# autowarefoundation/autoware_vision_pilot

Hardware: NVIDIA H100
Metric: camera frames/sec @1080p multi-task (higher is better)
Workload: dtype f16

## Files before the change

### autoware_vision_pilot_b200/_lib.py

```python
from __future__ import annotations

import ctypes as C
import os

import numpy as np

_HERE = os.path.dirname(os.path.abspath(__file__))
LIB_PATH = os.path.join(_HERE, "lib", "libvp_b200.so")

VPB_F16, VPB_BF16 = 0, 1
ACT_NONE, ACT_GELU, ACT_SILU, ACT_SIGMOID = 0, 1, 2, 3
EPI_STORE, EPI_ADD, EPI_MULADD, EPI_FINAL = 0, 1, 2, 3
FINAL_NONE, FINAL_ARGMAX, FINAL_THRESH, FINAL_EGOLANES = 0, 1, 2, 3
ALGO_TILE, ALGO_LINEAR = 0, 1


class ConvArgs(C.Structure):

    _fields_ = [
        ("dtype", C.c_int),
        ("H", C.c_int), ("W", C.c_int), ("Cin", C.c_int), ("ldi", C.c_int),
        ("Cout", C.c_int), ("taps", C.c_int), ("phases", C.c_int),
        ("act", C.c_int), ("mode", C.c_int), ("final_kind", C.c_int),
        ("inp", C.c_void_p), ("w", C.c_void_p), ("bias", C.c_void_p),
# ... 263 lines not shown
                ("bev_left_coeffs", C.c_double * 6), ("bev_right_coeffs", C.c_double * 6),
                ("bev_center_coeffs", C.c_double * 6),
                ("lane_offset", C.c_double), ("yaw_offset", C.c_double), ("curvature", C.c_double),
                ("bev_lane_offset", C.c_double), ("bev_yaw_offset", C.c_double), ("bev_curvature", C.c_double),
                ("last_valid_width_pixels", C.c_double),
                ("left_valid", C.c_int), ("right_valid", C.c_int), ("path_valid", C.c_int), ("bev_valid", C.c_int),
                ("filt_left_valid", C.c_int), ("filt_right_valid", C.c_int),
                ("left_start", C.c_int * 2), ("right_start", C.c_int * 2),
                ("n_left_pts", C.c_int), ("n_right_pts", C.c_int),
                ("pf_left_coeff", C.c_double * 3), ("pf_right_coeff", C.c_double * 3),
                ("pf_left_cte", C.c_double), ("pf_left_yaw_error", C.c_double),
                ("pf_right_cte", C.c_double), ("pf_right_yaw_error", C.c_double),
                ("pf_cte", C.c_double), ("pf_yaw_error", C.c_double), ("pf_curvature", C.c_double),
                ("pf_lane_width", C.c_double), ("pf_cte_variance", C.c_double), ("pf_yaw_variance", C.c_double),
                ("pf_curv_variance", C.c_double), ("pf_lane_width_variance", C.c_double),
                ("pf_fused_valid", C.c_int), ("pf_ran", C.c_int),
                ("pf_meas", (C.c_double * 2) * 14)]


_lib = None


def lib() -> C.CDLL:
    global _lib
    if _lib is None:
        if not os.path.exists(LIB_PATH):
            raise RuntimeError(
                f"{LIB_PATH} is missing — run `python -c 'import __graft_entry__ as g; g.build()'` "
                "(there is no CPU or PyTorch fallback for the B200 path)")
        _lib = C.CDLL(LIB_PATH)
        _lib.vpb_last_error.restype = C.c_char_p
        _lib.vpb_conv_gemm.argtypes = [C.POINTER(ConvArgs), C.c_void_p]
        _lib.vpb_conv_gemm.restype = C.c_int
    return _lib


def last_error() -> str:
    return lib().vpb_last_error().decode("utf-8", "replace")


def check(rc: int, what: str) -> None:
    if rc != 0:
        raise RuntimeError(f"{what} failed (rc={rc}): {last_error()}")
```

### autoware_vision_pilot_b200/csrc/conv_gemm.cu

```cuda
#include "common.cuh"
#include "conv_gemm.cuh"
#include "ops_internal.h"
#include <cstdio>
#include <cstring>
#include <algorithm>

namespace vpb {

static constexpr int kMma = 256;
static constexpr int kEpilogue = 128;
static constexpr int kThreads = kMma + kEpilogue + 32;
static constexpr int kMaxStages = 8;
static constexpr int kATileBytes = 128 * 128;
static constexpr int kMaxDynSmem = 227 * 1024 - 4096;
__host__ __device__ constexpr int acc_pitch(int bn) { return bn + 4; }
__host__ __device__ constexpr size_t acc_bytes(int bn) { return static_cast<size_t>(128) * acc_pitch(bn) * 4; }

__device__ __forceinline__ void acc_ld16(uint32_t t, uint32_t (&r)[16]) {
  const uint32_t a = t << 2;
#pragma unroll
  for (int i = 0; i < 4; ++i)
    asm volatile("ld.shared.v4.b32 {%0, %1, %2, %3}, [%4];"
                 : "=r"(r[4 * i]), "=r"(r[4 * i + 1]), "=r"(r[4 * i + 2]), "=r"(r[4 * i + 3])
                 : "r"(a + 16u * i)
// ... 179 lines not shown
    uint32_t ra[16];
    acc_ld16(ta, ra);
    finish(ra, sb4, op, rp);
  }
}

template <class E>
__device__ __forceinline__ void epilogue_tile(const ConvKParams& p, uint32_t t_row, int n0,
                                              const float* sbias, const EpiPix& px) {
  const bool whole = !p.split && n0 + p.BN <= p.nlim && p.act2 == ACT_NONE;
  if (whole && p.mode == VPB_EPI_STORE && p.act == ACT_GELU) epilogue_store_fast<E, ACT_GELU>(p, t_row, n0, sbias, px);
  else if (whole && p.mode == VPB_EPI_STORE && p.act == ACT_NONE) epilogue_store_fast<E, ACT_NONE>(p, t_row, n0, sbias, px);
  else if (whole && p.mode == VPB_EPI_STORE && p.act == ACT_SILU) epilogue_store_fast<E, ACT_SILU>(p, t_row, n0, sbias, px);
  else if (whole && p.mode == VPB_EPI_ADD && p.act == ACT_NONE && n0 + p.BN <= p.ldr) epilogue_store_fast<E, ACT_NONE, true>(p, t_row, n0, sbias, px);
  else epilogue_chunks<E>(p, t_row, n0, sbias, px);
}

struct TileCoord { int img, ph, n0, h0, w0; };

__device__ __forceinline__ TileCoord decode_tile(const ConvKParams& p, int tile) {
  TileCoord c;
  c.img = static_cast<int>(fast_div(tile, p.mg_ti));
  const int ti = tile - c.img * p.tiles_img;
  c.ph = static_cast<int>(fast_div(ti, p.mg_tpp));
  const int r = ti - c.ph * (p.tiles_n * p.tiles_h * p.tiles_w);
  const int rn = static_cast<int>(fast_div(r, p.mg_tn));
  const int thi = static_cast<int>(fast_div(rn, p.mg_tw));
  c.n0 = (r - rn * p.tiles_n) * p.BN;
  c.h0 = thi * p.TH;
  c.w0 = (rn - thi * p.tiles_w) * p.TW;
  return c;
}

template <class E, int BN>
__global__ void __launch_bounds__(kThreads, 1)
conv_wgmma_kernel(const __grid_constant__ ConvMaps maps, const ConvKParams p) {
  extern __shared__ uint8_t smem_raw[];
  __shared__ __align__(8) uint64_t bar_full[kMaxStages];
  __shared__ __align__(8) uint64_t bar_empty[kMaxStages];
  __shared__ __align__(8) uint64_t acc_full;
  __shared__ __align__(8) uint64_t acc_empty;
  __shared__ __align__(16) float s_bias[BN];

  constexpr uint32_t kBTileBytes = static_cast<uint32_t>(BN) * 128u;
  constexpr uint32_t kStageBytes = kATileBytes + kBTileBytes;
  constexpr int kPitch = acc_pitch(BN);
  const int warp = threadIdx.x >> 5;
  const int lane = threadIdx.x & 31;
  const uint32_t smem_base = (smem_u32(smem_raw) + 1023u) & ~1023u;
  const uint32_t acc_base = smem_base + static_cast<uint32_t>(p.stages) * kStageBytes;

  if (threadIdx.x == kMma + kEpilogue) {
    tma_prefetch_desc(&maps.A);
    tma_prefetch_desc(&maps.B);
    if (p.kchunks2) { tma_prefetch_desc(&maps.A2); tma_prefetch_desc(&maps.B2); }
    if (p.split) { tma_prefetch_desc(&maps.Alo); tma_prefetch_desc(&maps.Blo); }
    for (int s = 0; s < p.stages; ++s) {
      mbar_init(smem_u32(&bar_full[s]), 1);
      mbar_init(smem_u32(&bar_empty[s]), kMma / 32);
    }
    mbar_init(smem_u32(&acc_full), kMma);
    mbar_init(smem_u32(&acc_empty), kEpilogue);
    fence_mbar_init();
  }
  __syncthreads();
  pdl_launch_dependents();
  pdl_wait();

  const int nseg = p.split ? 3 : 1;
  const int kiters_all = p.upc ? 4 * p.kchunks + 9 * p.kchunks2 : (p.taps * p.kchunks + p.kchunks2) * nseg;

  if (warp == (kMma + kEpilogue) / 32) {
    int stage = 0;
    uint32_t phase = 0;
    auto load_stage = [&](const CUtensorMap* mA, int a0, int a1, int a2, int a3,
                          const CUtensorMap* mB, int b0, int b1, int b2) {
      mbar_wait_quiet(smem_u32(&bar_empty[stage]), phase ^ 1u);
      if (elect_one()) {
        const uint32_t full = smem_u32(&bar_full[stage]);
        const uint32_t sa = smem_base + stage * kStageBytes;
        mbar_arrive_expect_tx(full, kStageBytes);
        tma_load_4d(sa, mA, full, a0, a1, a2, a3);
        tma_load_3d(sa + kATileBytes, mB, full, b0, b1, b2);
      }
      __syncwarp();
      if (++stage == p.stages) { stage = 0; phase ^= 1u; }
    };
    for (int tile = blockIdx.x; tile < p.total_tiles; tile += gridDim.x) {
      const auto [img, ph, n0, h0, w0] = decode_tile(p, tile);
      if (p.upc) {
        const int pa = ph >> 1, pb = ph & 1;
        for (int t = 0; t < 4; ++t) {
          const int oy = (t >> 1) - 1 + pa, ox = (t & 1) - 1 + pb;
          for (int c = 0; c < p.kchunks; ++c)
            load_stage(&maps.A, c * 64, w0 + ox, h0 + oy, img, &maps.B, c * 64, n0, ph * 4 + t);
        }
        for (int t2 = 0; t2 < (p.kchunks2 ? 9 : 0); ++t2) {
          const int dy = t2 / 3, dx = t2 - dy * 3;
          const int u = pa + dy - 1, v = pb + dx - 1;
          for (int c2 = 0; c2 < p.kchunks2; ++c2)
            load_stage(&maps.A2, c2 * 64, 2 * w0 + v, 2 * h0 + u, img, &maps.B2, c2 * 64, n0, t2);
        }
        continue;
      }
      for (int t = 0; t < p.taps; ++t) {
        const int dy = (p.taps == 9) ? (t / 3 - 1) : 0;
        const int dx = (p.taps == 9) ? (t % 3 - 1) : 0;
        const int wsel = p.w_img ? img : (p.phases > 1) ? ph : t;
        for (int c = 0; c < p.kchunks; ++c)
          for (int seg = 0; seg < nseg; ++seg)
            load_stage(seg == 1 ? &maps.Alo : &maps.A, c * 64, w0 * p.stride + dx, h0 * p.stride + dy, img,
                       seg == 2 ? &maps.Blo : &maps.B, c * 64, n0, wsel);
      }
      const int s2 = p.phases > 1 ? 2 : 1;
      for (int c2 = 0; c2 < p.kchunks2; ++c2)
        for (int seg = 0; seg < nseg; ++seg)
          load_stage(seg == 1 ? &maps.A2lo : &maps.A2, c2 * 64, s2 * w0 + (ph & 1), s2 * h0 + (ph >> 1), img,
                     seg == 2 ? &maps.B2lo : &maps.B2, c2 * 64, n0, 0);
    }
  } else if (warp < kMma / 32) {
    const int wg = warp >> 2;
    float* acc_s = reinterpret_cast<float*>(smem_raw + (acc_base - smem_u32(smem_raw)));
    float acc[BN / 2];
    int stage = 0, prev = 0;
    uint32_t phase = 0, acc_phase = 0;
    for (int tile = blockIdx.x; tile < p.total_tiles; tile += gridDim.x) {
      for (int k = 0; k < kiters_all; ++k) {
        mbar_wait_quiet(smem_u32(&bar_full[stage]), phase);
        const uint32_t sa = smem_base + stage * kStageBytes;
        const uint64_t adesc = wgmma_desc_k128(sa + wg * (64 * 128));
        const uint64_t bdesc = wgmma_desc_k128(sa + kATileBytes);
        wgmma_fence();
#pragma unroll
        for (int kk = 0; kk < 4; ++kk)
          Wgmma<E, BN>::mma(acc, adesc + 2 * kk, bdesc + 2 * kk, (k | kk) != 0 ? 1u : 0u);
        wgmma_commit();
        wgmma_wait<1>();
        if (k > 0 && lane == 0) mbar_arrive(smem_u32(&bar_empty[prev]));
        prev = stage;
        if (++stage == p.stages) { stage = 0; phase ^= 1u; }
      }
      wgmma_wait<0>();
      if (lane == 0) mbar_arrive(smem_u32(&bar_empty[prev]));

      mbar_wait_quiet(smem_u32(&acc_empty), acc_phase ^ 1u);
      {
        const int r0 = wg * 64 + (warp & 3) * 16 + (lane >> 2);
        float* a0 = acc_s + r0 * kPitch + 2 * (lane & 3);
#pragma unroll
        for (int j = 0; j < BN / 8; ++j) {
          *reinterpret_cast<float2*>(a0 + 8 * j) = make_float2(acc[4 * j], acc[4 * j + 1]);
          *reinterpret_cast<float2*>(a0 + 8 * kPitch + 8 * j) = make_float2(acc[4 * j + 2], acc[4 * j + 3]);
        }
      }
      mbar_arrive(smem_u32(&acc_full));
      acc_phase ^= 1u;
    }
  } else {
    const int row = threadIdx.x - kMma;
    const int lh = row >> p.tw_shift;
    const int lw = row & (p.TW - 1);
    const int Wo = (p.phases > 1) ? 2 * p.W : p.W;
    const uint32_t t_row = (acc_base >> 2) + static_cast<uint32_t>(row * kPitch);
    uint32_t acc_phase = 0;
    for (int tile = blockIdx.x; tile < p.total_tiles; tile += gridDim.x) {
      const auto [img, ph, n0, h0, w0] = decode_tile(p, tile);
      const int h = h0 + lh, w = w0 + lw;

      named_bar_sync(1, kEpilogue);
      if (row < BN) {
        const int nn = n0 + row;
        s_bias[row] = (p.bias && nn < p.Cout) ? __ldg(p.bias + (p.upc ? 4 * p.Cout : 0) + nn) : 0.f;
      }
      named_bar_sync(1, kEpilogue);
      mbar_wait_quiet(smem_u32(&acc_full), acc_phase);

      const int oh = (p.phases > 1) ? 2 * h + (ph >> 1) : h;
      const int ow = (p.phases > 1) ? 2 * w + (ph & 1) : w;
      EpiPix px;
      px.ok = (h < p.H) && (w < p.W);
      px.ooff = img * p.out_img + static_cast<uint32_t>((oh + p.out_pad) * (Wo + 2 * p.out_pad) + (ow + p.out_pad)) * p.ldo;
      px.roff = img * p.res_img + static_cast<uint32_t>((oh + p.res_pad) * (Wo + 2 * p.res_pad) + (ow + p.res_pad)) * p.ldr;
      px.fpix = static_cast<uint32_t>(h * p.W + w);
      px.img = static_cast<uint32_t>(img);
      if (p.upc) {
        const int pa = ph >> 1, pb = ph & 1;
        const int cy = (pa == 0 && h == 0) ? 0 : (pa == 1 && h == p.H - 1) ? 2 : 1;
        const int cx = (pb == 0 && w == 0) ? 0 : (pb == 1 && w == p.W - 1) ? 2 : 1;
        const int cls = cy * 3 + cx;
        const float* gb = cls != 4 ? p.bias + cls * p.Cout + n0 : nullptr;
        if (p.act == ACT_GELU) epilogue_store_fast<E, ACT_GELU, false, true>(p, t_row, n0, s_bias, px, gb);
        else epilogue_store_fast<E, ACT_NONE, false, true>(p, t_row, n0, s_bias, px, gb);
      } else {
        epilogue_tile<E>(p, t_row, n0, s_bias, px);
      }
      mbar_arrive(smem_u32(&acc_empty));
      acc_phase ^= 1u;
    }
  }
}

__global__ void zero_border_kernel(uint4* out, int H, int W, int ldo, int nlim) {
  pdl_wait();
  out += (static_cast<size_t>(blockIdx.y) * (H + 2) * (W + 2) * ldo) >> 3;
  const int per = nlim >> 3, nb = 2 * (W + 2) + 2 * H;
  for (int i = blockIdx.x * blockDim.x + threadIdx.x; i < nb * per; i += gridDim.x * blockDim.x) {
    const int pix = i / per, v = i - pix * per;
    int y, x;
// ... 72 lines not shown
        q == cudaDriverEntryPointSuccess)
      fn = reinterpret_cast<EncodeTiledFn>(p);
  }
  return fn;
}

static int encode_map(CUtensorMap* m, const char* name, CUtensorMapDataType dt, int rank, const void* base,
                      const cuuint64_t* dims, const cuuint64_t* strides, const cuuint32_t* box, const cuuint32_t* es,
                      CUtensorMapL2promotion l2) {
  const CUresult r = get_encode_fn()(m, dt, rank, const_cast<void*>(base), dims, strides, box, es,
                                     CU_TENSOR_MAP_INTERLEAVE_NONE, CU_TENSOR_MAP_SWIZZLE_128B, l2,
                                     CU_TENSOR_MAP_FLOAT_OOB_FILL_NONE);
  if (r == CUDA_SUCCESS) return VPB_OK;
  vpb_set_error("conv: cuTensorMapEncodeTiled(%s) failed: %d", name, static_cast<int>(r));
  return VPB_ERR_CUDA;
}

int device_sm_count() {
  int dev = 0, n = 0;
  cudaGetDevice(&dev);
  cudaDeviceGetAttribute(&n, cudaDevAttrMultiProcessorCount, dev);
  return n > 0 ? n : 132;
}

static int pick_bn(int Cout, int want) {
  if (want > 0) return want <= 16 ? 16 : want <= 32 ? 32 : want <= 64 ? 64 : 128;
  for (int bn : {128, 64, 32}) {
    if (Cout <= bn && (Cout > bn / 2 || bn == 32)) return bn;
    if (Cout > bn && (Cout + bn - 1) / bn * bn - Cout <= Cout / 4) return bn;
  }
  return 16;
}

int conv_plan_build(const vpb_conv_args* a, ConvPlan* plan) {
  if (!a || !plan) return VPB_ERR_ARG;
  if (a->Cin <= 0 || (a->Cin & 7) || (a->ldi & 7) || a->ldi < a->Cin) {
    vpb_set_error("conv: Cin=%d ldi=%d must be multiples of 8 (ldi >= Cin)", a->Cin, a->ldi);
    return VPB_ERR_ARG;
  }
  const int cstride = a->stride == 2 ? 2 : 1;
  if (a->stride != 0 && a->stride != 1 && a->stride != 2) { vpb_set_error("conv: stride %d unsupported", a->stride); return VPB_ERR_ARG; }
  if (cstride == 2 && (a->algo == VPB_ALGO_LINEAR || a->phases != 1 || a->in_pad || a->in2 || a->in_lo)) {
    vpb_set_error("conv: stride 2 needs the TILE algorithm on an unpadded input, phases = 1, no second input");
    return VPB_ERR_ARG;
  }
  if (a->ldw != 0 && (a->ldw < a->Cin || (a->ldw & 7) || a->algo == VPB_ALGO_LINEAR)) {
    vpb_set_error("conv: ldw=%d must be a multiple of 8 >= Cin (TILE algorithm)", a->ldw);
    return VPB_ERR_ARG;
  }
  if (a->act2 != ACT_NONE && a->act2 != ACT_SILU) { vpb_set_error("conv: act2 supports SiLU only"); return VPB_ERR_ARG; }
  const bool upc = a->taps == 4 && a->phases == 4;
  if (upc && (a->algo == VPB_ALGO_LINEAR || a->in_lo || a->mode != VPB_EPI_STORE || (a->act != ACT_NONE && a->act != ACT_GELU) ||
              !a->bias || (a->Cout & 15) || a->out_slice || cstride != 1 || a->ldw || (a->in2 && a->taps2 != 9))) {
    vpb_set_error("conv: upconv (taps=4, phases=4) needs the TILE algorithm, 16-bit mode, STORE, act NONE|GELU, bias[9][Cout], Cout%%16==0, taps2=9 with in2");
    return VPB_ERR_ARG;
  }
  if (!((a->taps == 9 && a->phases == 1) || (a->taps == 1 && (a->phases == 1 || a->phases == 4)) || upc)) {
    vpb_set_error("conv: unsupported taps=%d phases=%d", a->taps, a->phases);
    return VPB_ERR_ARG;
  }
  const bool lin = a->algo == VPB_ALGO_LINEAR;
  if (lin && (a->taps != 9 || !a->in_pad)) {
    vpb_set_error("conv: the linear-padded algorithm needs a 3x3 conv on a zero-bordered input");
    return VPB_ERR_ARG;
  }
  if (a->mode == VPB_EPI_FINAL) {
    if (a->Cout > 32 || (a->out_cls && a->Cout > 16) || !a->out_f32) {
// ... 71 lines not shown
  }
  p.tiles_n = (a->Cout + p.BN - 1) / p.BN;
  p.kchunks = (a->Cin + 63) / 64;
  p.Cin2 = a->in2 ? a->Cin2 : 0;
  p.kchunks2 = (p.Cin2 + 63) / 64;
  int best_tw = 128; long best_cost = -1;
  for (int tw = 128; tw >= 8; tw >>= 1) {
    const int th = 128 / tw;
    const long cost = static_cast<long>((a->H + th - 1) / th) * ((a->W + tw - 1) / tw);
    if (best_cost < 0 || cost < best_cost) { best_cost = cost; best_tw = tw; }
  }
  p.TW = best_tw; p.TH = 128 / best_tw;
  p.tw_shift = 0; while ((1 << p.tw_shift) < p.TW) ++p.tw_shift;
  p.tiles_h = (a->H + p.TH - 1) / p.TH;
  p.tiles_w = (a->W + p.TW - 1) / p.TW;
  p.tiles_img = p.tiles_h * p.tiles_w * p.tiles_n * p.phases;
  p.total_tiles = p.tiles_img * batch;
  p.mg_ti = fast_div_magic(p.tiles_img);
  {
    const long ho = a->phases == 4 ? 2L * a->H : a->H, wo = a->phases == 4 ? 2L * a->W : a->W;
    p.out_img = static_cast<uint32_t>((ho + 2 * p.out_pad) * (wo + 2 * p.out_pad) * a->ldo);
    p.res_img = static_cast<uint32_t>((ho + 2 * p.res_pad) * (wo + 2 * p.res_pad) * a->ldr);
  }
  const size_t stage_bytes = kATileBytes + static_cast<size_t>(p.BN) * 128;
  p.stages = static_cast<int>(std::min<size_t>(kMaxStages, (kMaxDynSmem - 1024 - acc_bytes(p.BN)) / stage_bytes));
  if (p.stages < 2) { vpb_set_error("conv: no room for the operand ring (BN %d)", p.BN); return VPB_ERR_ARG; }
  plan->smem_bytes = p.stages * stage_bytes + acc_bytes(p.BN) + 1024;
  p.mg_tn = fast_div_magic(p.tiles_n); p.mg_tw = fast_div_magic(p.tiles_w);
  p.mg_tpp = fast_div_magic(p.tiles_n * p.tiles_h * p.tiles_w);
  p.act = a->act; p.mode = a->mode; p.final_kind = a->final_kind;
  p.bias = a->bias; p.out = a->out; p.ldo = a->ldo; p.res = a->res; p.ldr = a->ldr;
  p.out_f32 = a->out_f32; p.out_cls = a->out_cls;
  plan->dtype = a->dtype;
  plan->grid = std::min(p.total_tiles, device_sm_count());
  plan->flops = 2.0 * batch * a->H * a->W * static_cast<double>(a->Cout) * a->phases * (a->Cin * a->taps + p.Cin2 * (upc ? 9 : 1));

  const CUtensorMapDataType dt =
      a->dtype == VPB_BF16 ? CU_TENSOR_MAP_DATA_TYPE_BFLOAT16 : CU_TENSOR_MAP_DATA_TYPE_FLOAT16;
  ConvMaps& m = plan->maps;
  int rc;
  {
    const int pad = p.in_pad;
    const int Hin = (cstride == 2 && a->in_h > 0) ? a->in_h : a->H, Win = (cstride == 2 && a->in_w > 0) ? a->in_w : a->W;
    const size_t pitch = static_cast<size_t>(Win + 2 * pad) * a->ldi * 2;
    const size_t skip = pad * pitch + static_cast<size_t>(pad) * a->ldi * 2;
    const cuuint64_t dims[4] = {static_cast<cuuint64_t>(a->Cin), static_cast<cuuint64_t>(Win),
                                static_cast<cuuint64_t>(Hin), static_cast<cuuint64_t>(batch)};
    const cuuint64_t strides[3] = {static_cast<cuuint64_t>(a->ldi) * 2, pitch, pitch * (Hin + 2 * pad)};
    const cuuint32_t box[4] = {64, static_cast<cuuint32_t>(p.TW * cstride), static_cast<cuuint32_t>(p.TH * cstride), 1};
    const cuuint32_t es[4] = {1, static_cast<cuuint32_t>(cstride), static_cast<cuuint32_t>(cstride), 1};
    if ((rc = encode_map(&m.A, "A", dt, 4, static_cast<const uint8_t*>(a->in) + skip, dims, strides, box, es,
                         CU_TENSOR_MAP_L2_PROMOTION_L2_128B)))
      return rc;
    if (split && (rc = encode_map(&m.Alo, "Alo", dt, 4, static_cast<const uint8_t*>(a->in_lo) + skip, dims, strides, box,
                                  es, CU_TENSOR_MAP_L2_PROMOTION_L2_128B)))
      return rc;
  }
  {
    const size_t ldw = a->ldw > 0 ? a->ldw : a->Cin;
    const cuuint64_t dims[3] = {static_cast<cuuint64_t>(a->Cin), static_cast<cuuint64_t>(a->Cout),
                                static_cast<cuuint64_t>(a->w_img ? batch : a->taps * a->phases)};
    const cuuint64_t strides[2] = {static_cast<cuuint64_t>(ldw) * 2,
                                   a->w_img ? static_cast<cuuint64_t>(a->w_img) * 2 : static_cast<cuuint64_t>(ldw) * 2 * a->Cout};
    const cuuint32_t box[3] = {64, static_cast<cuuint32_t>(p.BN), 1};
    const cuuint32_t es[3] = {1, 1, 1};
    if ((rc = encode_map(&m.B, "B", dt, 3, a->w, dims, strides, box, es, CU_TENSOR_MAP_L2_PROMOTION_L2_256B))) return rc;
    if (split && (rc = encode_map(&m.Blo, "Blo", dt, 3, a->w_lo, dims, strides, box, es, CU_TENSOR_MAP_L2_PROMOTION_L2_256B)))
      return rc;
  }
  if (!split) { m.Alo = m.A; m.Blo = m.B; }
  m.A2 = m.A; m.B2 = m.B; m.A2lo = m.Alo; m.B2lo = m.Blo;
  if (a->in2) {
    const int s2 = a->phases == 4 ? 2 : 1;
    const int pad = a->in2_pad ? 1 : 0;
    const size_t px = static_cast<size_t>(a->ld2) * 2;
    const size_t pitch = static_cast<size_t>(a->W * s2 + 2 * pad) * px;
    const size_t skip = pad * pitch + pad * px;
    const cuuint64_t dims[4] = {static_cast<cuuint64_t>(a->Cin2), static_cast<cuuint64_t>(a->W * s2),
                                static_cast<cuuint64_t>(a->H * s2), static_cast<cuuint64_t>(batch)};
    const cuuint64_t strides[3] = {px, pitch, pitch * (a->H * s2 + 2 * pad)};
    const cuuint32_t box[4] = {64, static_cast<cuuint32_t>(p.TW * s2), static_cast<cuuint32_t>(p.TH * s2), 1};
    const cuuint32_t es[4] = {1, static_cast<cuuint32_t>(s2), static_cast<cuuint32_t>(s2), 1};
    if ((rc = encode_map(&m.A2, "A2", dt, 4, static_cast<const uint8_t*>(a->in2) + skip, dims, strides, box, es,
                         CU_TENSOR_MAP_L2_PROMOTION_L2_128B)))
      return rc;
    if (split && (rc = encode_map(&m.A2lo, "A2lo", dt, 4, static_cast<const uint8_t*>(a->in2_lo) + skip, dims, strides,
                                  box, es, CU_TENSOR_MAP_L2_PROMOTION_L2_128B)))
      return rc;
    const cuuint64_t bd[3] = {static_cast<cuuint64_t>(a->Cin2), static_cast<cuuint64_t>(a->Cout), static_cast<cuuint64_t>(p.upc ? 9 : 1)};
    const cuuint64_t bs[2] = {static_cast<cuuint64_t>(a->Cin2) * 2, static_cast<cuuint64_t>(a->Cin2) * 2 * a->Cout};
    const cuuint32_t bb[3] = {64, static_cast<cuuint32_t>(p.BN), 1};
    const cuuint32_t be[3] = {1, 1, 1};
    if ((rc = encode_map(&m.B2, "B2", dt, 3, a->w2, bd, bs, bb, be, CU_TENSOR_MAP_L2_PROMOTION_L2_256B))) return rc;
    if (split && (rc = encode_map(&m.B2lo, "B2lo", dt, 3, a->w2_lo, bd, bs, bb, be, CU_TENSOR_MAP_L2_PROMOTION_L2_256B)))
      return rc;
  }
  return VPB_OK;
}

static void (*const kConvKernels[2][4])(ConvMaps, ConvKParams) = {
    {conv_wgmma_kernel<F16, 16>, conv_wgmma_kernel<F16, 32>, conv_wgmma_kernel<F16, 64>, conv_wgmma_kernel<F16, 128>},
    {conv_wgmma_kernel<BF16, 16>, conv_wgmma_kernel<BF16, 32>, conv_wgmma_kernel<BF16, 64>, conv_wgmma_kernel<BF16, 128>},
};

int conv_plan_launch(const ConvPlan* plan, cudaStream_t stream) {
  {
    std::lock_guard<std::mutex> g(init_mutex());
    bool* done = device_flag(kInitConv);
    if (!*done) {
      for (const auto& by_bn : kConvKernels)
        for (const auto k : by_bn) VPB_CUDA_OK(cudaFuncSetAttribute(k, cudaFuncAttributeMaxDynamicSharedMemorySize, kMaxDynSmem));
      *done = true;
    }
  }
  const ConvKParams& p = plan->p;
  const auto kernel = kConvKernels[plan->dtype == VPB_BF16][__builtin_ctz(p.BN >> 4)];
  VPB_CUDA_OK(launch_k(kernel, dim3(plan->grid), dim3(kThreads), plan->smem_bytes, stream, plan->maps, p));
  if (p.lin) {
    const int n = (2 * (p.W + 2) + 2 * p.H) * (p.nlim >> 3);
    VPB_CUDA_OK(launch_k(zero_border_kernel, dim3(std::min((n + 255) / 256, 256), p.total_tiles / p.tiles_img), dim3(256), 0, stream,
                         static_cast<uint4*>(p.out), p.H, p.W, p.ldo, p.nlim));
  }
  return VPB_OK;
}

}


extern "C" int vpb_conv_gemm(const vpb_conv_args* a, void* stream) {
  vpb::ConvPlan plan;
  int rc = vpb::conv_plan_build(a, &plan);
  if (rc != VPB_OK) return rc;
  return vpb::conv_plan_launch(&plan, static_cast<cudaStream_t>(stream));
}

extern "C" int vpb_final_tapsum(const float* P, const float* bias, int Cout, int H, int W, int final_kind, float* out,
                                uint8_t* cls, int batch, void* stream) {
  return vpb::final_tapsum_x(P, bias, Cout, H, W, final_kind, out, cls, static_cast<cudaStream_t>(stream), batch);
}
```

### autoware_vision_pilot_b200/csrc/conv_gemm.cuh

```cuda
#pragma once
#include <cuda.h>
#include <cuda_runtime.h>
#include <stdint.h>
#include "../../include/vp_b200_ops.h"

namespace vpb {

struct ConvKParams {
  int H, W, Cin, Cout;
  int taps, phases;
  int TH, TW, tw_shift;
  int BN;
  int tiles_h, tiles_w, tiles_n;
  int total_tiles;
  int tiles_img;
  uint32_t mg_ti;
  uint32_t out_img, res_img;
  int kchunks;
  int Cin2, kchunks2;
  int stages;
  int lin;
  int upc;
  int nlim;
  int stride;
  int act2;
  int split;
  void* out_lo;
  const void* res_lo;
  int in_pad, out_pad, res_pad;
  uint32_t mg_tn, mg_tw, mg_tpp;
  int act, mode, final_kind;
  const float* bias;
  void* out;
  int ldo;
  const void* res;
  int ldr;
  float* out_f32;
  uint8_t* out_cls;
  int w_img;
};

struct ConvMaps {
  CUtensorMap A, B;
  CUtensorMap A2, B2;
  CUtensorMap Alo, Blo, A2lo, B2lo;
};

struct ConvPlan {
  ConvMaps maps;
  ConvKParams p;
  int dtype;
  int grid;
  size_t smem_bytes;
  double flops;
};

int conv_plan_build(const vpb_conv_args* a, ConvPlan* plan);
int conv_plan_launch(const ConvPlan* plan, cudaStream_t stream);
int device_sm_count();

}
```

### autoware_vision_pilot_b200/csrc/engine_common.cu

```cuda
#include "common.cuh"
#include "conv_gemm.cuh"
#include "engine_internal.h"

#include <algorithm>
#include <cstdio>
#include <cstdlib>
#include <cstring>

namespace vpb {

int load_vpw(const char* path, WeightMap& out) {
  FILE* fp = fopen(path, "rb");
  if (!fp) { vpb_set_error("cannot open weight file '%s'", path); return VPB_ERR_IO; }
  auto fail = [&](const char* why) { fclose(fp); vpb_set_error("%s: %s", path, why); return VPB_ERR_IO; };
  if (fseek(fp, 0, SEEK_END) != 0) return fail("cannot seek");
  const long file_size = ftell(fp);
  rewind(fp);
  char magic[4]; uint32_t n = 0;
  if (fread(magic, 1, 4, fp) != 4 || memcmp(magic, "VPW1", 4) != 0) return fail("not a VPW1 file");
  if (fread(&n, 4, 1, fp) != 1 || n > 100000) return fail("bad tensor count");
  for (uint32_t i = 0; i < n; ++i) {
    uint32_t nl = 0, dt = 0, nd = 0; uint64_t nb = 0;
    if (fread(&nl, 4, 1, fp) != 1 || nl > 4096) return fail("bad name length");
    std::string name(nl, '\0');
// ... 448 lines not shown
    if (op_events[i]) VPB_CUDA_OK(cudaEventRecord(op_events[i].get(), s));
  }
  for (size_t l = 1; l < nl; ++l) {
    if (!started[l]) continue;
    VPB_CUDA_OK(cudaEventRecord(lane_done[l].get(), lane_streams[l]));
    VPB_CUDA_OK(cudaStreamWaitEvent(st, lane_done[l].get(), 0));
  }
  for (size_t i = 0; i < ops.size() && rc == VPB_OK; ++i)
    if (ops[i].lane < 0) rc = launch_op(i, st);
  return rc;
}

vpb_conv_args EngineRuntime::conv_args(const Tens& in, const Tens* out, const Tens* res, int Cout, int taps, int phases,
                                       const void* w, const float* bias, int act, int mode, const Tens* in2,
                                       const void* w2) const {
  vpb_conv_args a{};
  a.batch = batch;
  a.dtype = dtype; a.H = in.H; a.W = in.W; a.Cin = in.C; a.ldi = in.ld;
  a.Cout = Cout; a.taps = taps; a.phases = phases; a.act = act; a.mode = mode;
  a.in = in.p; a.in_lo = in.lo; a.w = w; a.w_lo = lo(w); a.bias = bias;
  a.in_pad = in.pad;
  a.algo = (taps == 9 && in.pad && !split) ? VPB_ALGO_LINEAR : VPB_ALGO_TILE;
  if (out) { a.out = out->p; a.out_lo = out->lo; a.ldo = out->ld; a.out_pad = out->pad; }
  if (res) { a.res = res->p; a.res_lo = res->lo; a.ldr = res->ld; a.res_pad = res->pad; }
  if (in2) { a.in2 = in2->p; a.in2_lo = in2->lo; a.w2 = w2; a.w2_lo = lo(w2); a.Cin2 = in2->C; a.ld2 = in2->ld; a.in2_pad = in2->pad; }
  return a;
}

int EngineRuntime::append_conv(const std::string& name, const vpb_conv_args& a) {
  auto plan = std::make_unique<ConvPlan>();
  const int rc = conv_plan_build(&a, plan.get());
  if (rc != VPB_OK) { const std::string e = vpb_last_error(); vpb_set_error("%s: %s", name.c_str(), e.c_str()); return rc; }
  ConvPlan* pp = plan.get();
  plans.push_back(std::move(plan));
  conv_list.push_back(a);
  OpRec op; op.name = name; op.flops = pp->flops; op.gemm = true; op.lane = cur_lane;
  op.conv = static_cast<int>(plans.size()) - 1;
  op.kind = a.algo == VPB_ALGO_LINEAR ? 2 : 1;
  op.kname = "conv_wgmma_kernel";
  op.launch = [pp](cudaStream_t s) { return conv_plan_launch(pp, s); };
  ops.push_back(std::move(op));
  return VPB_OK;
}

int EngineRuntime::conv_args_of(int op, vpb_conv_args* out, const char** name, const char* who) const {
  if (!out) { vpb_set_error("%s: NULL output", who); return VPB_ERR_ARG; }
  if (op < 0 || op >= static_cast<int>(ops.size())) {
    vpb_set_error("%s: op %d out of range (the engine has %d ops)", who, op, static_cast<int>(ops.size()));
    return VPB_ERR_ARG;
  }
  if (ops[op].conv < 0) { vpb_set_error("%s: op %d (%s) is not a convolution", who, op, ops[op].name.c_str()); return VPB_ERR_ARG; }
  *out = conv_list[ops[op].conv];
  if (name) *name = ops[op].name.c_str();
  return VPB_OK;
}

bool frames_ok(const EngineRuntime* e, const vpb_frame_fmt* frames, int n, const char* who) {
  if (!e || !frames) { vpb_set_error("%s: bad arguments", who); return false; }
  if (n != e->batch) {
    vpb_set_error("%s: %d frame(s) for an engine of batch %d%s", who, n, e->batch,
                  n == 1 ? " (use the *_batch calls)" : "");
    return false;
  }
  for (int k = 0; k < n; ++k)
    if (frame_fmt_check(frames[k], who, k)) return false;
  return true;
// ... 242 lines not shown
```

### include/vp_b200_ops.h

```cpp
#ifndef VP_B200_OPS_H_
#define VP_B200_OPS_H_
#include <stddef.h>
#include <stdint.h>

#ifdef __cplusplus
extern "C" {
#endif

enum { VPB_OK = 0, VPB_ERR_ARG = -1, VPB_ERR_CUDA = -2, VPB_ERR_STATE = -3, VPB_ERR_IO = -4 };
enum { VPB_F16 = 0, VPB_BF16 = 1 };
enum { VPB_ACT_NONE = 0, VPB_ACT_GELU = 1, VPB_ACT_SILU = 2, VPB_ACT_SIGMOID = 3, VPB_ACT_SILU2 = 4  };
enum {
  VPB_EPI_STORE = 0,
  VPB_EPI_ADD = 1,
  VPB_EPI_MULADD = 2,
  VPB_EPI_FINAL = 3
};
enum {
  VPB_FINAL_NONE = 0,
  VPB_FINAL_ARGMAX = 1,
  VPB_FINAL_THRESH = 2,
  VPB_FINAL_EGOLANES = 3
};

// ... 28 lines not shown
  void* out;
  int ldo;
  const void* res;
  int ldr;
  float* out_f32;
  uint8_t* out_cls;
  int bn;
  int in_pad, out_pad, res_pad;
  int algo;
  int dbg_ms;
  int dbg_gb;
  int dbg_base_offset;
  const void* in2;
  const void* w2;
  int Cin2, ld2, in2_pad;
  int dbg_pair;
  int dbg_splitk;
  unsigned long long* dbg_trace;
  int stride, in_h, in_w;
  int ldw;
  int act2;
  int out_slice;
  const void* in_lo;
  const void* w_lo;
  void* out_lo;
  const void* res_lo;
  const void* in2_lo;
  const void* w2_lo;
  int taps2;
  int batch;
  int w_img;
} vpb_conv_args;
int vpb_conv_gemm(const vpb_conv_args* a, void* stream);
int vpb_final_tapsum(const float* P, const float* bias, int Cout, int H, int W, int final_kind, float* out,
                     uint8_t* cls, int batch, void* stream);
int vpb_final_conv_weights_host(const float* w, int Cout, int Cin, float* out);
int vpb_upconv_compose(const float* w3, const float* b3, const float* wt, const float* bt, const float* ws,
                       const float* bs, int Cout, int Cmid, int Cin, int C2, float* wf, float* w2f, float* bias9,
                       void* stream);
int vpb_f32_to_16(int dtype, const float* src, void* dst, long long n, void* stream);

enum { VPB_RESIZE_NONE = 0, VPB_RESIZE_PIL_BICUBIC = 1, VPB_RESIZE_CV_LINEAR = 2,
       VPB_RESIZE_PIL_BILINEAR = 3  };
enum { VPB_CONV_RGB = 0, VPB_CONV_BGR_NOSWAP = 1, VPB_CONV_BGR_SWAP = 2,
       VPB_CONV_RGB_UNIT = 3  };
int vpb_preprocess(const uint8_t* src_dev, int h, int w, int stride, int resize_mode, int convention,
                   int dtype, void* out_dev, uint8_t* out_u8_dev, void* stream);
int vpb_preprocess_fmt(const vpb_frame_fmt* frame_dev, int resize_mode, int convention, int dtype, void* out_dev,
                       uint8_t* out_u8_dev, void* stream);

typedef struct vpb_rectify vpb_rectify;
int  vpb_rectify_create(const int16_t* map1, const uint16_t* map2, int map_h, int map_w, int src_h, int src_w,
                        int gpu_id, vpb_rectify** out);
void vpb_rectify_destroy(vpb_rectify* r);
int  vpb_rectify_frames(const vpb_frame_fmt* frames_dev, const vpb_rectify* const* rect, int n, int bgr,
                        uint8_t* const* out, void* stream);
enum { VPB_JPEG_444 = 0, VPB_JPEG_422 = 1, VPB_JPEG_420 = 2 };
int vpb_jpeg_info(const uint8_t* data, size_t bytes, int* h, int* w, int* sampling);
typedef struct vpb_jpeg_decoder vpb_jpeg_decoder;
int  vpb_jpeg_decoder_create(int max_h, int max_w, int max_n, int gpu_id, vpb_jpeg_decoder** out);
void vpb_jpeg_decoder_destroy(vpb_jpeg_decoder* d);
int  vpb_jpeg_decode(vpb_jpeg_decoder* d, const vpb_frame_fmt* frames_host, int n, int bgr, uint8_t* const* out_dev,
                     void* stream);
int vpb_resize_tables_host(int mode, int in_size, int out_size, int* bounds, int* coeffs,
                           int coeffs_cap, int* ksize);

// ... 100 lines not shown
```

Measured before the change: 431.8.

## Add split-K to the conv WGMMA kernel with atomic-counter reduction in the epilogue

Each conv tile's K iterations can now be split across several CTAs. Each split writes a partial fp32 tile to a global workspace, and the last-arriving split, found through an atomic counter, sums the partials through the stage ring and runs the normal epilogue. A cost heuristic picks the split count automatically when the tile count would leave SMs idle. This is meant to fill the GPU on low-resolution, deep-channel layers, in exchange for workspace traffic, an extra sync between the loader and epilogue, and per-op workspace allocations.

```diff
diff --git a/autoware_vision_pilot_b200/_lib.py b/autoware_vision_pilot_b200/_lib.py
--- a/autoware_vision_pilot_b200/_lib.py
+++ b/autoware_vision_pilot_b200/_lib.py
@@ -319,6 +319,9 @@
         _lib.vpb_last_error.restype = C.c_char_p
         _lib.vpb_conv_gemm.argtypes = [C.POINTER(ConvArgs), C.c_void_p]
         _lib.vpb_conv_gemm.restype = C.c_int
+        _lib.vpb_conv_splitk_sizes.argtypes = [C.POINTER(ConvArgs), C.c_int, C.POINTER(C.c_int),
+                                               C.POINTER(C.c_size_t), C.POINTER(C.c_size_t)]
+        _lib.vpb_conv_gemm_splitk.argtypes = [C.POINTER(ConvArgs), C.c_int, C.c_void_p, C.c_void_p, C.c_void_p]
     return _lib
 
 
diff --git a/autoware_vision_pilot_b200/csrc/conv_gemm.cu b/autoware_vision_pilot_b200/csrc/conv_gemm.cu
--- a/autoware_vision_pilot_b200/csrc/conv_gemm.cu
+++ b/autoware_vision_pilot_b200/csrc/conv_gemm.cu
@@ -235,7 +235,53 @@
   return c;
 }
 
-template <class E, int BN>
+__device__ __forceinline__ float4 ld_shared_f4(uint32_t a) {
+  float4 v;
+  asm volatile("ld.shared.v4.f32 {%0, %1, %2, %3}, [%4];" : "=f"(v.x), "=f"(v.y), "=f"(v.z), "=f"(v.w) : "r"(a) : "memory");
+  return v;
+}
+
+template <int BN>
+__device__ __forceinline__ bool splitk_reduce(const ConvKParams& p, int tile, int s, float* acc_s, int row,
+                                              uint32_t* s_last, uint32_t ring, uint32_t ring_bytes) {
+  constexpr int kPitch = acc_pitch(BN), kRow4 = BN / 4, kSlot4 = 128 * kRow4;
+  const float4* ws = reinterpret_cast<const float4*>(p.ws) + static_cast<size_t>(tile) * p.splits * kSlot4;
+  for (int i = row; i < kSlot4; i += kEpilogue) {
+    const int r = i / kRow4, c = i - r * kRow4;
+    __stcg(const_cast<float4*>(ws) + s * kSlot4 + i, *reinterpret_cast<const float4*>(acc_s + r * kPitch + 4 * c));
+  }
+  named_bar_sync(1, kEpilogue);
+  if (row == 0) {
+    uint32_t before;
+    asm volatile("atom.acq_rel.gpu.global.add.u32 %0, [%1], 1;" : "=r"(before) : "l"(p.counters + tile) : "memory");
+    *s_last = before == static_cast<uint32_t>(p.splits - 1);
+  }
+  named_bar_sync(1, kEpilogue);
+  if (!*s_last) return false;
+  const int per_round = static_cast<int>(ring_bytes / (kSlot4 * 16u));
+  for (int j0 = 0; j0 < p.splits; j0 += per_round) {
+    const int m = min(per_round, p.splits - j0);
+    for (int i = row; i < m * kSlot4; i += kEpilogue)
+      asm volatile("cp.async.cg.shared.global [%0], [%1], 16;" :: "r"(ring + 16u * i), "l"(ws + j0 * kSlot4 + i) : "memory");
+    asm volatile("cp.async.commit_group;\n\tcp.async.wait_group 0;" ::: "memory");
+    named_bar_sync(1, kEpilogue);
+    for (int i = row; i < kSlot4; i += kEpilogue) {
+      const int r = i / kRow4, c = i - r * kRow4;
+      float4* dst = reinterpret_cast<float4*>(acc_s + r * kPitch + 4 * c);
+      float4 v = j0 == 0 ? ld_shared_f4(ring + 16u * i) : *dst;
+      for (int jj = j0 == 0 ? 1 : 0; jj < m; ++jj) {
+        const float4 q = ld_shared_f4(ring + 16u * (jj * kSlot4 + i));
+        v.x += q.x; v.y += q.y; v.z += q.z; v.w += q.w;
+      }
+      *dst = v;
+    }
+    named_bar_sync(1, kEpilogue);
+  }
+  if (row == 0) p.counters[tile] = 0u;
+  return true;
+}
+
+template <class E, int BN, bool SPLIT>
 __global__ void __launch_bounds__(kThreads, 1)
 conv_wgmma_kernel(const __grid_constant__ ConvMaps maps, const ConvKParams p) {
   extern __shared__ uint8_t smem_raw[];
@@ -243,7 +289,9 @@
   __shared__ __align__(8) uint64_t bar_empty[kMaxStages];
   __shared__ __align__(8) uint64_t acc_full;
   __shared__ __align__(8) uint64_t acc_empty;
+  __shared__ __align__(8) uint64_t ring_free;
   __shared__ __align__(16) float s_bias[BN];
+  __shared__ uint32_t s_last;
 
   constexpr uint32_t kBTileBytes = static_cast<uint32_t>(BN) * 128u;
   constexpr uint32_t kStageBytes = kATileBytes + kBTileBytes;
@@ -264,6 +312,7 @@
     }
     mbar_init(smem_u32(&acc_full), kMma);
     mbar_init(smem_u32(&acc_empty), kEpilogue);
+    mbar_init(smem_u32(&ring_free), 1);
     fence_mbar_init();
   }
   __syncthreads();
@@ -272,12 +321,18 @@
 
   const int nseg = p.split ? 3 : 1;
   const int kiters_all = p.upc ? 4 * p.kchunks + 9 * p.kchunks2 : (p.taps * p.kchunks + p.kchunks2) * nseg;
+  const int splits = SPLIT ? p.splits : 1;
+  const int total_units = p.total_tiles * splits;
+  auto k_begin = [&](int s) { return s * kiters_all / splits; };
 
   if (warp == (kMma + kEpilogue) / 32) {
     int stage = 0;
     uint32_t phase = 0;
+    int kpos = 0, kb = 0, ke = 0;
     auto load_stage = [&](const CUtensorMap* mA, int a0, int a1, int a2, int a3,
                           const CUtensorMap* mB, int b0, int b1, int b2) {
+      if (SPLIT && (kpos < kb || kpos >= ke)) { ++kpos; return; }
+      ++kpos;
       mbar_wait_quiet(smem_u32(&bar_empty[stage]), phase ^ 1u);
       if (elect_one()) {
         const uint32_t full = smem_u32(&bar_full[stage]);
@@ -289,7 +344,15 @@
       __syncwarp();
       if (++stage == p.stages) { stage = 0; phase ^= 1u; }
     };
-    for (int tile = blockIdx.x; tile < p.total_tiles; tile += gridDim.x) {
+    uint32_t ring_phase = 0;
+    for (int u = blockIdx.x; u < total_units; u += gridDim.x) {
+      const int tile = u / splits;
+      const int s = u - tile * splits;
+      kpos = 0; kb = k_begin(s); ke = k_begin(s + 1);
+      if (SPLIT && u != static_cast<int>(blockIdx.x)) {
+        mbar_wait_quiet(smem_u32(&ring_free), ring_phase);
+        ring_phase ^= 1u;
+      }
       const auto [img, ph, n0, h0, w0] = decode_tile(p, tile);
       if (p.upc) {
         const int pa = ph >> 1, pb = ph & 1;
@@ -300,9 +363,9 @@
         }
         for (int t2 = 0; t2 < (p.kchunks2 ? 9 : 0); ++t2) {
           const int dy = t2 / 3, dx = t2 - dy * 3;
-          const int u = pa + dy - 1, v = pb + dx - 1;
+          const int uu = pa + dy - 1, vv = pb + dx - 1;
           for (int c2 = 0; c2 < p.kchunks2; ++c2)
-            load_stage(&maps.A2, c2 * 64, 2 * w0 + v, 2 * h0 + u, img, &maps.B2, c2 * 64, n0, t2);
+            load_stage(&maps.A2, c2 * 64, 2 * w0 + vv, 2 * h0 + uu, img, &maps.B2, c2 * 64, n0, t2);
         }
         continue;
       }
@@ -327,8 +390,10 @@
     float acc[BN / 2];
     int stage = 0, prev = 0;
     uint32_t phase = 0, acc_phase = 0;
-    for (int tile = blockIdx.x; tile < p.total_tiles; tile += gridDim.x) {
-      for (int k = 0; k < kiters_all; ++k) {
+    for (int u = blockIdx.x; u < total_units; u += gridDim.x) {
+      const int s = u % splits;
+      const int kb = k_begin(s);
+      for (int k = kb, ke = k_begin(s + 1); k < ke; ++k) {
         mbar_wait_quiet(smem_u32(&bar_full[stage]), phase);
         const uint32_t sa = smem_base + stage * kStageBytes;
         const uint64_t adesc = wgmma_desc_k128(sa + wg * (64 * 128));
@@ -336,10 +401,10 @@
         wgmma_fence();
 #pragma unroll
         for (int kk = 0; kk < 4; ++kk)
-          Wgmma<E, BN>::mma(acc, adesc + 2 * kk, bdesc + 2 * kk, (k | kk) != 0 ? 1u : 0u);
+          Wgmma<E, BN>::mma(acc, adesc + 2 * kk, bdesc + 2 * kk, (k != kb || kk != 0) ? 1u : 0u);
         wgmma_commit();
         wgmma_wait<1>();
-        if (k > 0 && lane == 0) mbar_arrive(smem_u32(&bar_empty[prev]));
+        if (k > kb && lane == 0) mbar_arrive(smem_u32(&bar_empty[prev]));
         prev = stage;
         if (++stage == p.stages) { stage = 0; phase ^= 1u; }
       }
@@ -365,8 +430,10 @@
     const int lw = row & (p.TW - 1);
     const int Wo = (p.phases > 1) ? 2 * p.W : p.W;
     const uint32_t t_row = (acc_base >> 2) + static_cast<uint32_t>(row * kPitch);
+    float* acc_s = reinterpret_cast<float*>(smem_raw + (acc_base - smem_u32(smem_raw)));
     uint32_t acc_phase = 0;
-    for (int tile = blockIdx.x; tile < p.total_tiles; tile += gridDim.x) {
+    for (int u = blockIdx.x; u < total_units; u += gridDim.x) {
+      const int tile = u / splits;
       const auto [img, ph, n0, h0, w0] = decode_tile(p, tile);
       const int h = h0 + lh, w = w0 + lw;
 
@@ -377,6 +444,18 @@
       }
       named_bar_sync(1, kEpilogue);
       mbar_wait_quiet(smem_u32(&acc_full), acc_phase);
+      if constexpr (SPLIT) {
+        const bool last = splitk_reduce<BN>(p, tile, u - tile * splits, acc_s, row, &s_last, smem_base,
+                                            static_cast<uint32_t>(p.stages) * kStageBytes);
+        fence_proxy_async();
+        named_bar_sync(1, kEpilogue);
+        if (row == 0) mbar_arrive(smem_u32(&ring_free));
+        if (!last) {
+          mbar_arrive(smem_u32(&acc_empty));
+          acc_phase ^= 1u;
+          continue;
+        }
+      }
 
       const int oh = (p.phases > 1) ? 2 * h + (ph >> 1) : h;
       const int ow = (p.phases > 1) ? 2 * w + (ph & 1) : w;
@@ -515,7 +594,29 @@
   return 16;
 }
 
-int conv_plan_build(const vpb_conv_args* a, ConvPlan* plan) {
+static constexpr int kMaxSplits = 8;
+static constexpr double kSplitFixup = 14.0;
+
+int conv_pick_splits(int tiles, int chunks, int sms) {
+  int best = 1;
+  double best_cost = static_cast<double>((tiles + sms - 1) / sms) * chunks;
+  for (int s = 2; s <= std::min(kMaxSplits, chunks); ++s) {
+    const double cost = static_cast<double>((tiles * s + sms - 1) / sms) * (static_cast<double>(chunks) / s + kSplitFixup * s);
+    if (cost < best_cost) { best = s; best_cost = cost; }
+  }
+  return best;
+}
+
+size_t conv_ws_bytes(const ConvPlan& plan) {
+  const ConvKParams& p = plan.p;
+  return p.splits > 1 ? static_cast<size_t>(p.total_tiles) * p.splits * 128 * p.BN * sizeof(float) : 0;
+}
+
+size_t conv_counter_bytes(const ConvPlan& plan) {
+  return plan.p.splits > 1 ? static_cast<size_t>(plan.p.total_tiles) * sizeof(unsigned) : 0;
+}
+
+int conv_plan_build(const vpb_conv_args* a, ConvPlan* plan, int splits) {
   if (!a || !plan) return VPB_ERR_ARG;
   if (a->Cin <= 0 || (a->Cin & 7) || (a->ldi & 7) || a->ldi < a->Cin) {
     vpb_set_error("conv: Cin=%d ldi=%d must be multiples of 8 (ldi >= Cin)", a->Cin, a->ldi);
@@ -653,7 +754,13 @@
   p.bias = a->bias; p.out = a->out; p.ldo = a->ldo; p.res = a->res; p.ldr = a->ldr;
   p.out_f32 = a->out_f32; p.out_cls = a->out_cls;
   plan->dtype = a->dtype;
-  plan->grid = std::min(p.total_tiles, device_sm_count());
+  {
+    const int nseg = split ? 3 : 1;
+    const int kiters = upc ? 4 * p.kchunks + 9 * p.kchunks2 : (p.taps * p.kchunks + p.kchunks2) * nseg;
+    if (splits < 0 || splits > kMaxSplits) { vpb_set_error("conv: splits %d outside 0..%d", splits, kMaxSplits); return VPB_ERR_ARG; }
+    p.splits = (split || lin) ? 1 : splits > 0 ? std::min(splits, kiters) : conv_pick_splits(p.tiles_img, kiters, device_sm_count());
+  }
+  plan->grid = std::min(p.total_tiles * p.splits, device_sm_count());
   plan->flops = 2.0 * batch * a->H * a->W * static_cast<double>(a->Cout) * a->phases * (a->Cin * a->taps + p.Cin2 * (upc ? 9 : 1));
 
   const CUtensorMapDataType dt =
@@ -719,9 +826,15 @@
   return VPB_OK;
 }
 
-static void (*const kConvKernels[2][4])(ConvMaps, ConvKParams) = {
-    {conv_wgmma_kernel<F16, 16>, conv_wgmma_kernel<F16, 32>, conv_wgmma_kernel<F16, 64>, conv_wgmma_kernel<F16, 128>},
-    {conv_wgmma_kernel<BF16, 16>, conv_wgmma_kernel<BF16, 32>, conv_wgmma_kernel<BF16, 64>, conv_wgmma_kernel<BF16, 128>},
+static void (*const kConvKernels[2][2][4])(ConvMaps, ConvKParams) = {
+    {{conv_wgmma_kernel<F16, 16, false>, conv_wgmma_kernel<F16, 32, false>, conv_wgmma_kernel<F16, 64, false>,
+      conv_wgmma_kernel<F16, 128, false>},
+     {conv_wgmma_kernel<BF16, 16, false>, conv_wgmma_kernel<BF16, 32, false>, conv_wgmma_kernel<BF16, 64, false>,
+      conv_wgmma_kernel<BF16, 128, false>}},
+    {{conv_wgmma_kernel<F16, 16, true>, conv_wgmma_kernel<F16, 32, true>, conv_wgmma_kernel<F16, 64, true>,
+      conv_wgmma_kernel<F16, 128, true>},
+     {conv_wgmma_kernel<BF16, 16, true>, conv_wgmma_kernel<BF16, 32, true>, conv_wgmma_kernel<BF16, 64, true>,
+      conv_wgmma_kernel<BF16, 128, true>}},
 };
 
 int conv_plan_launch(const ConvPlan* plan, cudaStream_t stream) {
@@ -729,13 +842,15 @@
     std::lock_guard<std::mutex> g(init_mutex());
     bool* done = device_flag(kInitConv);
     if (!*done) {
-      for (const auto& by_bn : kConvKernels)
-        for (const auto k : by_bn) VPB_CUDA_OK(cudaFuncSetAttribute(k, cudaFuncAttributeMaxDynamicSharedMemorySize, kMaxDynSmem));
+      for (const auto& by_dtype : kConvKernels)
+        for (const auto& by_bn : by_dtype)
+          for (const auto k : by_bn) VPB_CUDA_OK(cudaFuncSetAttribute(k, cudaFuncAttributeMaxDynamicSharedMemorySize, kMaxDynSmem));
       *done = true;
     }
   }
   const ConvKParams& p = plan->p;
-  const auto kernel = kConvKernels[plan->dtype == VPB_BF16][__builtin_ctz(p.BN >> 4)];
+  if (p.splits > 1 && (!p.ws || !p.counters)) { vpb_set_error("conv: a split-K plan needs its workspace and counters"); return VPB_ERR_ARG; }
+  const auto kernel = kConvKernels[p.splits > 1][plan->dtype == VPB_BF16][__builtin_ctz(p.BN >> 4)];
   VPB_CUDA_OK(launch_k(kernel, dim3(plan->grid), dim3(kThreads), plan->smem_bytes, stream, plan->maps, p));
   if (p.lin) {
     const int n = (2 * (p.W + 2) + 2 * p.H) * (p.nlim >> 3);
@@ -748,11 +863,46 @@
 }
 
 
+extern "C" int vpb_conv_splitk_sizes(const vpb_conv_args* a, int splits, int* used, size_t* ws_bytes,
+                                     size_t* counter_bytes) {
+  vpb::ConvPlan plan;
+  const int rc = vpb::conv_plan_build(a, &plan, splits);
+  if (rc != VPB_OK) return rc;
+  if (used) *used = plan.p.splits;
+  if (ws_bytes) *ws_bytes = vpb::conv_ws_bytes(plan);
+  if (counter_bytes) *counter_bytes = vpb::conv_counter_bytes(plan);
+  return VPB_OK;
+}
+
+extern "C" int vpb_conv_gemm_splitk(const vpb_conv_args* a, int splits, void* ws, void* counters, void* stream) {
+  vpb::ConvPlan plan;
+  int rc = vpb::conv_plan_build(a, &plan, splits);
+  if (rc != VPB_OK) return rc;
+  const cudaStream_t st = static_cast<cudaStream_t>(stream);
+  const size_t wsb = vpb::conv_ws_bytes(plan), cb = vpb::conv_counter_bytes(plan);
+  if (!wsb) return vpb::conv_plan_launch(&plan, st);
+  if ((ws != nullptr) != (counters != nullptr)) { vpb_set_error("conv: give both ws and counters, or neither"); return VPB_ERR_ARG; }
+  if (ws) {
+    plan.p.ws = static_cast<float*>(ws);
+    plan.p.counters = static_cast<unsigned*>(counters);
+    return vpb::conv_plan_launch(&plan, st);
+  }
+  void* buf = nullptr;
+  VPB_CUDA_OK(cudaMallocAsync(&buf, wsb + cb, st));
+  plan.p.ws = static_cast<float*>(buf);
+  plan.p.counters = reinterpret_cast<unsigned*>(static_cast<uint8_t*>(buf) + wsb);
+  if (cudaMemsetAsync(plan.p.counters, 0, cb, st) != cudaSuccess) {
+    vpb_set_error("conv: zeroing the split-K counters failed");
+    rc = VPB_ERR_CUDA;
+  } else {
+    rc = vpb::conv_plan_launch(&plan, st);
+  }
+  cudaFreeAsync(buf, st);
+  return rc;
+}
+
 extern "C" int vpb_conv_gemm(const vpb_conv_args* a, void* stream) {
-  vpb::ConvPlan plan;
-  int rc = vpb::conv_plan_build(a, &plan);
-  if (rc != VPB_OK) return rc;
-  return vpb::conv_plan_launch(&plan, static_cast<cudaStream_t>(stream));
+  return vpb_conv_gemm_splitk(a, 0, nullptr, nullptr, stream);
 }
 
 extern "C" int vpb_final_tapsum(const float* P, const float* bias, int Cout, int H, int W, int final_kind, float* out,
diff --git a/autoware_vision_pilot_b200/csrc/conv_gemm.cuh b/autoware_vision_pilot_b200/csrc/conv_gemm.cuh
--- a/autoware_vision_pilot_b200/csrc/conv_gemm.cuh
+++ b/autoware_vision_pilot_b200/csrc/conv_gemm.cuh
@@ -38,6 +38,9 @@
   float* out_f32;
   uint8_t* out_cls;
   int w_img;
+  int splits;
+  float* ws;
+  unsigned* counters;
 };
 
 struct ConvMaps {
@@ -55,8 +58,11 @@
   double flops;
 };
 
-int conv_plan_build(const vpb_conv_args* a, ConvPlan* plan);
+int conv_plan_build(const vpb_conv_args* a, ConvPlan* plan, int splits = 0);
 int conv_plan_launch(const ConvPlan* plan, cudaStream_t stream);
+int conv_pick_splits(int tiles, int chunks, int sms);
+size_t conv_ws_bytes(const ConvPlan& plan);
+size_t conv_counter_bytes(const ConvPlan& plan);
 int device_sm_count();
 
 }
diff --git a/autoware_vision_pilot_b200/csrc/engine_common.cu b/autoware_vision_pilot_b200/csrc/engine_common.cu
--- a/autoware_vision_pilot_b200/csrc/engine_common.cu
+++ b/autoware_vision_pilot_b200/csrc/engine_common.cu
@@ -504,6 +504,11 @@
   const int rc = conv_plan_build(&a, plan.get());
   if (rc != VPB_OK) { const std::string e = vpb_last_error(); vpb_set_error("%s: %s", name.c_str(), e.c_str()); return rc; }
   ConvPlan* pp = plan.get();
+  if (const size_t wsb = conv_ws_bytes(*pp)) {
+    pp->p.ws = static_cast<float*>(dalloc(wsb));
+    pp->p.counters = static_cast<unsigned*>(dalloc(conv_counter_bytes(*pp)));
+    if (!pp->p.ws || !pp->p.counters) return VPB_ERR_CUDA;
+  }
   plans.push_back(std::move(plan));
   conv_list.push_back(a);
   OpRec op; op.name = name; op.flops = pp->flops; op.gemm = true; op.lane = cur_lane;
diff --git a/include/vp_b200_ops.h b/include/vp_b200_ops.h
--- a/include/vp_b200_ops.h
+++ b/include/vp_b200_ops.h
@@ -84,6 +84,8 @@
   int w_img;
 } vpb_conv_args;
 int vpb_conv_gemm(const vpb_conv_args* a, void* stream);
+int vpb_conv_splitk_sizes(const vpb_conv_args* a, int splits, int* used, size_t* ws_bytes, size_t* counter_bytes);
+int vpb_conv_gemm_splitk(const vpb_conv_args* a, int splits, void* ws, void* counters, void* stream);
 int vpb_final_tapsum(const float* P, const float* bias, int Cout, int H, int W, int final_kind, float* out,
                      uint8_t* cls, int batch, void* stream);
 int vpb_final_conv_weights_host(const float* w, int Cout, int Cin, float* out);
```

After: 427.8, median of 6. About the same (-0.9%).
